# taishan1994/pytorch-distributed-NLP

Hardware: NVIDIA H100
Metric: training samples/sec (seq_len=128) (higher is better)
Workload: dtype bf16

## Files before the change

### pytorch-distributed-nlp_b200/csrc/gemm.cu

```cuda
#include "common.cuh"
#include "gemm_epilogue.cuh"
#include "../../include/b2_ddp_bert.h"

namespace b2 {

constexpr int BM = 128;
constexpr int BK = 64;
constexpr int WGMMA_K = 16;
constexpr int kGemmThreads = (4 + kEpiWarps) * 32;

template <int BN>
struct GemmCfg {
  static constexpr int kABytes = BM * BK * 2;
  static constexpr int kBBytes = BN * BK * 2;
  static constexpr int kStageBytes = kABytes + kBBytes;
  static constexpr int kStages = (BN == 256) ? 4 : 6;
  static constexpr int kPipeBytes = kStages * kStageBytes;
  static constexpr int kAccLd = BN + 4;
  static constexpr int kSmemBytes = kPipeBytes + kEpiWarps * kEpiStageBytes + 1024  + 256 ;
  static_assert(BM * kAccLd * 4 <= kPipeBytes, "the accumulator tile lives in the drained operand ring");
};

template <int BN, bool A_MN, bool B_MN>
__device__ __forceinline__ void gemm_mainloop(uint8_t* smem, uint64_t* full_bar, uint64_t* empty_bar,
                                              const CUtensorMap* tmap_a, const CUtensorMap* tmap_b, int m0, int n0,
                                              int kb0, int kb1, int warp, int lane) {
  using Cfg = GemmCfg<BN>;
  if (warp == 0) {
    if (lane == 0) {
      int stage = 0; uint32_t phase = 0;
      for (int kb = kb0; kb < kb1; ++kb) {
        mbar_wait(&empty_bar[stage], phase ^ 1);
        mbar_expect_tx(&full_bar[stage], Cfg::kStageBytes);
        uint8_t* sa = smem + stage * Cfg::kStageBytes;
        uint8_t* sb = sa + Cfg::kABytes;
        const int k0 = kb * BK;
        if (!A_MN) {
          tma_load_2d(sa, tmap_a, &full_bar[stage], k0, m0);
        } else {
#pragma unroll
          for (int j = 0; j < BM / 64; ++j)
            tma_load_2d(sa + j * (BK * 128), tmap_a, &full_bar[stage], m0 + 64 * j, k0);
        }
        if (!B_MN) {
          tma_load_2d(sb, tmap_b, &full_bar[stage], k0, n0);
        } else {
#pragma unroll
          for (int j = 0; j < BN / 64; ++j)
            tma_load_2d(sb + j * (BK * 128), tmap_b, &full_bar[stage], n0 + 64 * j, k0);
        }
        if (++stage == Cfg::kStages) { stage = 0; phase ^= 1; }
      }
    }
  } else if (warp >= 4) {
    const int wg = (warp - 4) >> 2;
    constexpr uint32_t a_lbo = A_MN ? BK * 128 : 16, b_lbo = B_MN ? BK * 128 : 16;
    constexpr uint32_t a_kstep = A_MN ? WGMMA_K * 128 : WGMMA_K * 2;
    constexpr uint32_t b_kstep = B_MN ? WGMMA_K * 128 : WGMMA_K * 2;
    float acc[BN / 2];
#pragma unroll
    for (int i = 0; i < BN / 2; ++i) acc[i] = 0.f;
    int stage = 0, prev = -1; uint32_t phase = 0;
    for (int kb = kb0; kb < kb1; ++kb) {
      mbar_wait(&full_bar[stage], phase);
      const uint32_t sa = smem_u32(smem + stage * Cfg::kStageBytes) + wg * 8192;
      const uint32_t sb = smem_u32(smem + stage * Cfg::kStageBytes + Cfg::kABytes);
      wgmma_fence();
#pragma unroll
      for (int k = 0; k < BK / WGMMA_K; ++k)
        wgmma_bf16<BN, A_MN ? 1 : 0, B_MN ? 1 : 0>(acc, make_smem_desc(sa + k * a_kstep, a_lbo, 1024),
                                                     make_smem_desc(sb + k * b_kstep, b_lbo, 1024),
                                                     (kb > kb0 || k > 0) ? 1u : 0u);
      wgmma_commit();
      wgmma_wait<1>();
      if (prev >= 0 && lane == 0) mbar_arrive(&empty_bar[prev]);
      prev = stage;
      if (++stage == Cfg::kStages) { stage = 0; phase ^= 1; }
    }
    wgmma_wait<0>();
    wgmma_fence_regs(acc);
    if (prev >= 0 && lane == 0) mbar_arrive(&empty_bar[prev]);
    named_barrier_sync(1, kEpiWarps * 32);
    float* accs = reinterpret_cast<float*>(smem);
    const int r = wg * 64 + (warp & 3) * 16 + (lane >> 2);
    const int c = 2 * (lane & 3);
#pragma unroll
    for (int j = 0; j < BN / 8; ++j) {
      *reinterpret_cast<float2*>(accs + (size_t)r * Cfg::kAccLd + 8 * j + c) = make_float2(acc[4 * j], acc[4 * j + 1]);
      *reinterpret_cast<float2*>(accs + (size_t)(r + 8) * Cfg::kAccLd + 8 * j + c) =
          make_float2(acc[4 * j + 2], acc[4 * j + 3]);
    }
    named_barrier_sync(1, kEpiWarps * 32);
  }
}

template <int BN>
__device__ __forceinline__ void gemm_setup(uint64_t* full_bar, uint64_t* empty_bar) {
  if (threadIdx.x == 0) {
    for (int s = 0; s < GemmCfg<BN>::kStages; ++s) {
      mbar_init(&full_bar[s], 1);
      mbar_init(&empty_bar[s], kEpiWarps);
    }
    fence_mbar_init();
  }
  __syncthreads();
}

template <int BN, bool A_MN, bool B_MN>
__global__ void __launch_bounds__(kGemmThreads, 1)
gemm_bf16_kernel(const __grid_constant__ CUtensorMap tmap_a, const __grid_constant__ CUtensorMap tmap_b,
                 const GemmKernelParams p) {
  using Cfg = GemmCfg<BN>;
  extern __shared__ uint8_t smem_raw[];
  uint8_t* smem = smem_align_1024(smem_raw);
  uint8_t* epi_stage = smem + Cfg::kPipeBytes;
  uint64_t* full_bar = reinterpret_cast<uint64_t*>(epi_stage + kEpiWarps * kEpiStageBytes);
  uint64_t* empty_bar = full_bar + Cfg::kStages;
  const int warp = threadIdx.x >> 5;
  const int lane = threadIdx.x & 31;
  if (threadIdx.x == 0) {
    tma_prefetch_desc(&tmap_a);
    tma_prefetch_desc(&tmap_b);
  }
  gemm_setup<BN>(full_bar, empty_bar);
  pdl_wait();
  pdl_launch_dependents();

  const int tile = blockIdx.x / p.splits, split = blockIdx.x % p.splits;
  const int m0 = (tile / p.tiles_n) * BM, n0 = (tile % p.tiles_n) * BN;
  const int kb0 = split * p.kblocks_per_split;
  const int kb1 = min(kb0 + p.kblocks_per_split, p.kblocks_total);
  gemm_mainloop<BN, A_MN, B_MN>(smem, full_bar, empty_bar, &tmap_a, &tmap_b, m0, n0, kb0, kb1, warp, lane);
  if (warp >= 4) {
    const DropCtx drop = make_drop_ctx(p.rng, p.rng_site, p.dropout_p);
    epilogue_tile<BN>(p, drop, reinterpret_cast<const float*>(smem), Cfg::kAccLd, warp, lane, m0, n0, split,
                      epi_stage + (warp - 4) * kEpiStageBytes);
  }
}

constexpr int kMaxGroup = 4;
struct GroupedProblem {
  int M, N, tiles_n, tile_begin;
  __nv_bfloat16* D; long long ldd;
};
struct GroupedParams {
  int count, num_work, kblocks;
  GroupedProblem pr[kMaxGroup];
};

struct GroupedMaps {
  CUtensorMap a[kMaxGroup], b[kMaxGroup];
};
__device__ __forceinline__ int grouped_find(const GroupedParams& gp, int w) {
  int pi = 0;
#pragma unroll
  for (int i = 1; i < kMaxGroup; ++i)
    if (i < gp.count && w >= gp.pr[i].tile_begin) pi = i;
  return pi;
}

__global__ void __launch_bounds__(kGemmThreads, 1)
gemm_grouped_tn_kernel(const __grid_constant__ GroupedMaps maps, const GroupedParams gp) {
  constexpr int BN = 256;
  using Cfg = GemmCfg<BN>;
  extern __shared__ uint8_t smem_raw[];
  uint8_t* smem = smem_align_1024(smem_raw);
  uint8_t* epi_stage = smem + Cfg::kPipeBytes;
  uint64_t* full_bar = reinterpret_cast<uint64_t*>(epi_stage + kEpiWarps * kEpiStageBytes);
  uint64_t* empty_bar = full_bar + Cfg::kStages;
  const int warp = threadIdx.x >> 5;
  const int lane = threadIdx.x & 31;
  const int pi = grouped_find(gp, blockIdx.x);
  if (threadIdx.x == 0) {
    tma_prefetch_desc(&maps.a[pi]);
    tma_prefetch_desc(&maps.b[pi]);
  }
  gemm_setup<BN>(full_bar, empty_bar);
  pdl_wait();
  pdl_launch_dependents();

  const GroupedProblem& pr = gp.pr[pi];
  const int lt = blockIdx.x - pr.tile_begin;
  const int m0 = (lt / pr.tiles_n) * BM;
  const int n0 = (lt % pr.tiles_n) * BN;
  gemm_mainloop<BN, true, true>(smem, full_bar, empty_bar, &maps.a[pi], &maps.b[pi], m0, n0, 0, gp.kblocks, warp,
                                lane);
  if (warp < 4) return;
  uint8_t* stage = epi_stage + (warp - 4) * kEpiStageBytes;
  GemmKernelParams q;
  q.splits = 1; q.epilogue = B2_EPI_NONE; q.bias = nullptr; q.aux_in = nullptr; q.aux_out = nullptr;
  q.partial = nullptr; q.dropout_p = 0.f; q.rng = nullptr; q.rng_site = 0; q.timing = nullptr; q.colsum = nullptr;
  q.ld_aux_in = 0; q.ld_aux_out = 0; q.K = 0; q.tiles_m = 0; q.kblocks_per_split = 0; q.kblocks_total = 0;
  q.M = pr.M; q.N = pr.N; q.tiles_n = pr.tiles_n; q.D = pr.D; q.ldd = pr.ldd;
  DropCtx drop;
  drop.k0 = 0; drop.k1 = 0; drop.step = 0; drop.site = 0; drop.thresh = 0; drop.scale = 1.f;
  epilogue_tile<BN>(q, drop, reinterpret_cast<const float*>(smem), Cfg::kAccLd, warp, lane, m0, n0, 0, stage);
}

__global__ void splitk_reduce_kernel(const float* __restrict__ partial, __nv_bfloat16* __restrict__ D,
                                     long long ldd, int M, int N, int splits) {
  pdl_wait();
  pdl_launch_dependents();
  const long long idx = (long long)blockIdx.x * blockDim.x + threadIdx.x;
  const long long total = (long long)M * N / 4;
  if (idx >= total) return;
  const long long e = idx * 4;
  const int m = (int)(e / N), n = (int)(e % N);
  float4 acc = make_float4(0.f, 0.f, 0.f, 0.f);
  for (int s = 0; s < splits; ++s) {
    const float4 v = *reinterpret_cast<const float4*>(partial + (size_t)s * M * N + e);
    acc.x += v.x; acc.y += v.y; acc.z += v.z; acc.w += v.w;
  }
  uint2 o;
  o.x = pack_bf16(acc.x, acc.y);
  o.y = pack_bf16(acc.z, acc.w);
  *reinterpret_cast<uint2*>(D + (size_t)m * ldd + n) = o;
}

static int g_num_sms = 0;
static int num_sms() {
  if (g_num_sms == 0) {
    int dev = 0;
    cudaGetDevice(&dev);
    cudaDeviceGetAttribute(&g_num_sms, cudaDevAttrMultiProcessorCount, dev);
    if (g_num_sms <= 0) g_num_sms = 132;
  }
  return g_num_sms;
}

static void fill_params(GemmKernelParams& p, const b2_gemm_args_t& a, int tile_m, int bn, int splits) {
  p.M = (int)a.M; p.N = (int)a.N; p.K = (int)a.K;
  p.tiles_m = (p.M + tile_m - 1) / tile_m;
  p.tiles_n = (p.N + bn - 1) / bn;
  p.kblocks_total = (p.K + BK - 1) / BK;
  p.splits = splits;
  p.kblocks_per_split = (p.kblocks_total + splits - 1) / splits;
  p.epilogue = (splits > 1 && a.epilogue != B2_EPI_ACCUM_F32) ? B2_EPI_PARTIAL_F32 : a.epilogue;
  p.D = (__nv_bfloat16*)a.D; p.ldd = a.ldd;
  p.bias = (const __nv_bfloat16*)a.bias;
  p.aux_in = (const __nv_bfloat16*)a.aux_in; p.ld_aux_in = a.ld_aux_in;
  p.aux_out = (__nv_bfloat16*)a.aux_out; p.ld_aux_out = a.ld_aux_out;
  p.partial = (float*)a.workspace;
  p.dropout_p = a.dropout_p; p.rng = (const unsigned long long*)a.rng_state; p.rng_site = a.rng_site;
  p.timing = (long long*)a.debug_timing;
  p.colsum = a.colsum_out;
}

static int32_t launch_splitk_reduce(const b2_gemm_args_t& a, int splits, cudaStream_t stream) {
  const long long total = (long long)a.M * a.N / 4;
  B2_LAUNCH(splitk_reduce_kernel, (unsigned)((total + 255) / 256), 256, 0, stream, 
      (const float*)a.workspace, (__nv_bfloat16*)a.D, a.ldd, (int)a.M, (int)a.N, splits);
  B2_CUDA(cudaGetLastError());
  count_launches(1);
  return 0;
}

template <int BN, bool A_MN, bool B_MN>
static int32_t launch_gemm(const b2_gemm_args_t& a, int splits, cudaStream_t stream) {
  using Cfg = GemmCfg<BN>;
  CUtensorMap ta, tb;
  int32_t st;
  if (!A_MN) st = get_tensor_map_2d(&ta, a.A, (uint64_t)a.M, (uint64_t)a.K, (uint64_t)a.lda * 2, BM, 64);
  else       st = get_tensor_map_2d(&ta, a.A, (uint64_t)a.K, (uint64_t)a.M, (uint64_t)a.lda * 2, BK, 64);
  if (st) return st;
  if (!B_MN) st = get_tensor_map_2d(&tb, a.B, (uint64_t)a.N, (uint64_t)a.K, (uint64_t)a.ldb * 2, BN, 64);
  else       st = get_tensor_map_2d(&tb, a.B, (uint64_t)a.K, (uint64_t)a.N, (uint64_t)a.ldb * 2, BK, 64);
  if (st) return st;
  GemmKernelParams p;
  fill_params(p, a, BM, BN, splits);
  auto kern = gemm_bf16_kernel<BN, A_MN, B_MN>;
  static bool attr_set = false;
  if (!attr_set) {
    B2_CUDA(cudaFuncSetAttribute(kern, cudaFuncAttributeMaxDynamicSharedMemorySize, Cfg::kSmemBytes));
    attr_set = true;
  }
  const int work = p.tiles_m * p.tiles_n * p.splits;
  B2_LAUNCH(kern, work, kGemmThreads, Cfg::kSmemBytes, stream, ta, tb, p);
  B2_CUDA(cudaGetLastError());
  count_launches(1);
  if (splits > 1 && a.epilogue != B2_EPI_ACCUM_F32) return launch_splitk_reduce(a, splits, stream);
  return 0;
}

struct Choice { int bn, splits; };
static Choice choose_config(const b2_gemm_args_t& a) {
  const int sms = num_sms();
  const int kblocks = (int)((a.K + BK - 1) / BK);
  const bool accum = a.epilogue == B2_EPI_ACCUM_F32;
  const bool can_split = accum || ((a.epilogue == B2_EPI_NONE) && a.workspace != nullptr && a.bias == nullptr &&
                                   a.colsum_out == nullptr);
  double best = 1e30;
  Choice c{128, 1};
  const double l2_bytes_per_cycle = 3000.0;
  const int bns[2] = {256, 128};
  for (int bi = 0; bi < 2; ++bi) {
    const int bn = bns[bi];
    if (a.N % bn != 0 && bn != 128) continue;
    const int tiles = (int)((a.M + BM - 1) / BM) * (int)((a.N + bn - 1) / bn);
    const int max_s = can_split ? 8 : 1;
    for (int s = 1; s <= max_s; s = accum ? s + 1 : s * 2) {
      if (s > 1 && (kblocks / s < 8)) break;
      if (s > 1 && !accum && (size_t)s * a.M * a.N * 4 > (size_t)a.workspace_bytes) break;
      const int work = tiles * s;
      const int rounds = (work + sms - 1) / sms;
      const int busy_sms = work < sms ? work : sms;
      const double mma_cycles = 128.0 * bn * 64 / 2048.0;
      const double bytes_per_sm = (128 + bn) * 128.0;
      const double feed_cycles = bytes_per_sm * busy_sms / l2_bytes_per_cycle;
      const double kb_cycles = mma_cycles > feed_cycles ? mma_cycles : feed_cycles;
      double t = rounds * ((double)((kblocks + s - 1) / s) * kb_cycles + 2500.0 );
      if (s > 1 && !accum) t += 1500.0 + (double)s * a.M * a.N * 8 / 3000.0;
      if (s > 1 && accum) t += (double)(s - 1) * a.M * a.N * 4 / 3000.0;
      if (t < best) { best = t; c = Choice{bn, s}; }
    }
  }
  return c;
}

}

using namespace b2;

static int32_t check_args(const b2_gemm_args_t* a) {
  B2_REQUIRE(a != nullptr, "b2_gemm_bf16: null args");
  B2_REQUIRE(a->M > 0 && a->N > 0 && a->K > 0, "b2_gemm_bf16: empty problem M=%lld N=%lld K=%lld",
             (long long)a->M, (long long)a->N, (long long)a->K);
  B2_REQUIRE(a->A && a->B && a->D, "b2_gemm_bf16: null operand pointer");
  B2_REQUIRE(a->N % 64 == 0, "b2_gemm_bf16: N=%lld must be a multiple of 64", (long long)a->N);
  B2_REQUIRE(a->K % 8 == 0 && a->lda % 8 == 0 && a->ldb % 8 == 0 && a->ldd % 8 == 0,
             "b2_gemm_bf16: K and leading dimensions must be multiples of 8 elements (16 B)");
  B2_REQUIRE(((uintptr_t)a->A % 16 == 0) && ((uintptr_t)a->B % 16 == 0) && ((uintptr_t)a->D % 16 == 0),
             "b2_gemm_bf16: operands must be 16-byte aligned");
  const int64_t a_row = a->a_major == B2_MAJOR_MN ? a->M : a->K, b_row = a->b_major == B2_MAJOR_MN ? a->N : a->K;
  B2_REQUIRE(a->lda >= a_row, "b2_gemm_bf16: lda=%lld is below the row it describes (%lld)", (long long)a->lda,
             (long long)a_row);
  B2_REQUIRE(a->ldb >= b_row, "b2_gemm_bf16: ldb=%lld is below the row it describes (%lld)", (long long)a->ldb,
             (long long)b_row);
  B2_REQUIRE(a->ldd >= a->N, "b2_gemm_bf16: ldd=%lld is below N=%lld", (long long)a->ldd, (long long)a->N);
  const int e = a->epilogue;
  B2_REQUIRE(e >= B2_EPI_NONE && e <= B2_EPI_ACCUM_F32, "b2_gemm_bf16: bad epilogue %d", e);
  const bool with_bias = e == B2_EPI_BIAS || e == B2_EPI_BIAS_GELU || e == B2_EPI_BIAS_DROPOUT_RESIDUAL;
  const bool f32_out = e == B2_EPI_RESIDUAL_F32 || e == B2_EPI_ACCUM_F32;
  if (with_bias) B2_REQUIRE(a->bias != nullptr, "b2_gemm_bf16: epilogue %d needs a bias", e);
  else           B2_REQUIRE(a->bias == nullptr, "b2_gemm_bf16: epilogue %d adds no bias: bias must be NULL", e);
  if (e == B2_EPI_BIAS_DROPOUT_RESIDUAL || e == B2_EPI_RESIDUAL || e == B2_EPI_GELU_BWD || e == B2_EPI_RESIDUAL_F32) {
    B2_REQUIRE(a->aux_in != nullptr && a->ld_aux_in % 8 == 0, "b2_gemm_bf16: epilogue %d needs aux_in", e);
    B2_REQUIRE(a->ld_aux_in >= a->N, "b2_gemm_bf16: ld_aux_in=%lld is below N=%lld", (long long)a->ld_aux_in,
               (long long)a->N);
  }
  if (e == B2_EPI_BIAS_GELU) {
    B2_REQUIRE(a->aux_out != nullptr && a->ld_aux_out % 8 == 0, "b2_gemm_bf16: BIAS_GELU needs aux_out");
    B2_REQUIRE(a->ld_aux_out >= a->N, "b2_gemm_bf16: ld_aux_out=%lld is below N=%lld", (long long)a->ld_aux_out,
               (long long)a->N);
  } else
    B2_REQUIRE(a->aux_out == nullptr, "b2_gemm_bf16: only BIAS_GELU writes aux_out: aux_out must be NULL");
  B2_REQUIRE((uintptr_t)a->bias % 16 == 0, "b2_gemm_bf16: bias must be 16-byte aligned");
  B2_REQUIRE((uintptr_t)a->aux_in % 16 == 0, "b2_gemm_bf16: aux_in must be 16-byte aligned");
  B2_REQUIRE((uintptr_t)a->aux_out % 16 == 0, "b2_gemm_bf16: aux_out must be 16-byte aligned");
  B2_REQUIRE(a->dropout_p >= 0.f && a->dropout_p < 1.f, "b2_gemm_bf16: dropout_p out of range");
  if (e == B2_EPI_BIAS_DROPOUT_RESIDUAL && a->dropout_p > 0.f)
    B2_REQUIRE(a->rng_state != nullptr, "b2_gemm_bf16: dropout needs rng_state");
  if (e != B2_EPI_BIAS_DROPOUT_RESIDUAL)
    B2_REQUIRE(a->dropout_p == 0.f, "b2_gemm_bf16: epilogue %d applies no dropout: dropout_p must be 0", e);
  B2_REQUIRE(a->colsum_out == nullptr || !f32_out, "b2_gemm_bf16: epilogue %d has no bf16 output: colsum_out must be "
             "NULL", e);
  B2_REQUIRE(a->colsum_out == nullptr || a->force_splits <= 1, "b2_gemm_bf16: colsum_out needs force_splits <= 1");
  if (a->force_bn == 128 || a->force_bn == 256)
    B2_REQUIRE(a->N % a->force_bn == 0 || a->force_bn == 128, "b2_gemm_bf16: force_bn does not divide N");
  if (a->force_splits > 1)
    B2_REQUIRE(e == B2_EPI_ACCUM_F32 ||
                   (e == B2_EPI_NONE && a->workspace &&
                    (size_t)a->force_splits * a->M * a->N * 4 <= (size_t)a->workspace_bytes),
               "b2_gemm_bf16: split-K needs EPI_ACCUM_F32, or EPI_NONE and a large enough workspace");
  B2_REQUIRE(!(a->a_major == B2_MAJOR_MN && a->b_major != B2_MAJOR_MN),
             "b2_gemm_bf16: layout TT (A MN-major, B K-major) is not on the path");
  return 0;
}

static int32_t launch_checked(const b2_gemm_args_t* a, cudaStream_t stream) {
  Choice c = choose_config(*a);
  if (a->force_bn == 128 || a->force_bn == 256) c.bn = a->force_bn;
  if (a->force_splits >= 1) c.splits = a->force_splits;
  const bool a_mn = a->a_major == B2_MAJOR_MN, b_mn = a->b_major == B2_MAJOR_MN;

#define B2_DISPATCH(BN_)                                                          \
  if (c.bn == BN_) {                                                              \
    if (!a_mn && !b_mn) return launch_gemm<BN_, false, false>(*a, c.splits, stream); \
    if (!a_mn && b_mn) return launch_gemm<BN_, false, true>(*a, c.splits, stream);   \
    return launch_gemm<BN_, true, true>(*a, c.splits, stream);                       \
  }
  B2_DISPATCH(128)
  B2_DISPATCH(256)
#undef B2_DISPATCH
  set_error("b2_gemm_bf16: no kernel for BN=%d", c.bn);
  return -2;
}

extern "C" int32_t b2_gemm_bf16(const b2_gemm_args_t* a, void* stream_) {
  const int32_t st = check_args(a);
  if (st) return st;
  return launch_checked(a, (cudaStream_t)stream_);
}

extern "C" int32_t b2_gemm_bf16_grouped(const b2_gemm_args_t* args, int32_t count, void* stream_) {
  cudaStream_t stream = (cudaStream_t)stream_;
  B2_REQUIRE(args != nullptr && count >= 1, "b2_gemm_bf16_grouped: no problems");
  for (int i = 0; i < count; ++i) {
    const int32_t st = check_args(&args[i]);
    if (st) return st;
  }
  bool groupable = count <= kMaxGroup;
  for (int i = 0; i < count && groupable; ++i) {
    const b2_gemm_args_t& a = args[i];
    groupable = a.a_major == B2_MAJOR_MN && a.b_major == B2_MAJOR_MN && a.epilogue == B2_EPI_NONE &&
                a.colsum_out == nullptr && a.N % 256 == 0 && a.K == args[0].K && a.force_splits <= 1 &&
                (a.force_bn == 0 || a.force_bn == 256);
  }
  if (!groupable) {
    for (int i = 0; i < count; ++i) {
      const int32_t st = launch_checked(&args[i], stream);
      if (st) return st;
    }
    return 0;
  }
  GroupedMaps maps;
  GroupedParams gp;
  gp.count = count;
  gp.kblocks = (int)((args[0].K + BK - 1) / BK);
  int work = 0;
  for (int i = 0; i < count; ++i) {
    const b2_gemm_args_t& a = args[i];
    int32_t st = get_tensor_map_2d(&maps.a[i], a.A, (uint64_t)a.K, (uint64_t)a.M, (uint64_t)a.lda * 2, BK, 64);
    if (st) return st;
    st = get_tensor_map_2d(&maps.b[i], a.B, (uint64_t)a.K, (uint64_t)a.N, (uint64_t)a.ldb * 2, BK, 64);
    if (st) return st;
    GroupedProblem& g = gp.pr[i];
    g.M = (int)a.M; g.N = (int)a.N; g.tiles_n = (int)(a.N / 256); g.tile_begin = work;
    g.D = (__nv_bfloat16*)a.D; g.ldd = a.ldd;
    work += (int)((a.M + BM - 1) / BM) * g.tiles_n;
  }
  for (int i = count; i < kMaxGroup; ++i) { gp.pr[i] = gp.pr[0]; gp.pr[i].tile_begin = 0x7fffffff; maps.a[i] = maps.a[0]; maps.b[i] = maps.b[0]; }
  gp.num_work = work;
  static bool attr_set = false;
  if (!attr_set) {
    B2_CUDA(cudaFuncSetAttribute(gemm_grouped_tn_kernel, cudaFuncAttributeMaxDynamicSharedMemorySize,
                                 GemmCfg<256>::kSmemBytes));
    attr_set = true;
  }
  B2_LAUNCH(gemm_grouped_tn_kernel, work, kGemmThreads, GemmCfg<256>::kSmemBytes, stream, maps, gp);
  B2_CUDA(cudaGetLastError());
  count_launches(1);
  return 0;
}
```

### pytorch-distributed-nlp_b200/csrc/gemm_epilogue.cuh

```cuda
#pragma once
#include "common.cuh"
#include "../../include/b2_ddp_bert.h"

namespace b2 {

struct GemmKernelParams {
  int M, N, K;
  int tiles_m, tiles_n, splits, kblocks_per_split, kblocks_total;
  int epilogue;
  __nv_bfloat16* D; long long ldd;
  const __nv_bfloat16* bias;
  const __nv_bfloat16* aux_in; long long ld_aux_in;
  __nv_bfloat16* aux_out; long long ld_aux_out;
  float* partial;
  float dropout_p; const unsigned long long* rng; unsigned rng_site;
  long long* timing;
  float* colsum;
};

constexpr int kEpiStageBytes = 32 * 128;

#ifdef __CUDACC__
template <int CH>
__device__ __forceinline__ uint4* stage_ptr(uint8_t* stage, int row, int chunk) {
  if (CH == 8) return reinterpret_cast<uint4*>(stage + row * 128 + ((chunk ^ (row & 7)) << 4));
  return reinterpret_cast<uint4*>(stage + (row >> 1) * 128 + (((((row & 1) << 2) | chunk) ^ ((row >> 1) & 7)) << 4));
}
template <int CH>
__device__ __forceinline__ void tile_s2g(uint8_t* stage, uint8_t* g, long long pitch, int lane, int rows_valid) {
  constexpr int RPS = 32 / CH;
#pragma unroll
  for (int k = 0; k < CH; ++k) {
    const int r = RPS * k + lane / CH, c = lane % CH;
    const uint4 v = *stage_ptr<CH>(stage, r, c);
    if (r < rows_valid) *reinterpret_cast<uint4*>(g + (size_t)r * pitch + c * 16) = v;
  }
}
__device__ __forceinline__ void tile_s2g_red_f32(uint8_t* stage, uint8_t* g, long long pitch, int lane,
                                                 int rows_valid) {
#pragma unroll
  for (int k = 0; k < 8; ++k) {
    const int r = 4 * k + (lane >> 3), c = lane & 7;
    const uint4 v = *stage_ptr<8>(stage, r, c);
    if (r < rows_valid)
      asm volatile("red.global.add.v4.f32 [%0], {%1, %2, %3, %4};" ::"l"(g + (size_t)r * pitch + c * 16),
                   "f"(__uint_as_float(v.x)), "f"(__uint_as_float(v.y)), "f"(__uint_as_float(v.z)),
                   "f"(__uint_as_float(v.w))
                   : "memory");
  }
}
template <int CH>
__device__ __forceinline__ void tile_g2s_async(uint8_t* stage, const uint8_t* g, long long pitch, int lane,
                                               int rows_valid) {
  constexpr int RPS = 32 / CH;
#pragma unroll
  for (int k = 0; k < CH; ++k) {
    const int r = RPS * k + lane / CH, c = lane % CH;
    uint4* dst = stage_ptr<CH>(stage, r, c);
    if (r < rows_valid) {
      asm volatile("cp.async.cg.shared.global [%0], [%1], 16;" ::"r"(smem_u32(dst)), "l"(g + (size_t)r * pitch + c * 16)
                   : "memory");
    } else {
      *dst = make_uint4(0u, 0u, 0u, 0u);
    }
  }
  asm volatile("cp.async.commit_group;" ::: "memory");
}
__device__ __forceinline__ void tile_async_wait() { asm volatile("cp.async.wait_group 0;" ::: "memory"); }

__device__ __forceinline__ void acc_ld32(const float* a, uint32_t (&v)[32]) {
#pragma unroll
  for (int k = 0; k < 8; ++k) {
    const uint4 t = *reinterpret_cast<const uint4*>(a + 4 * k);
    v[4 * k] = t.x; v[4 * k + 1] = t.y; v[4 * k + 2] = t.z; v[4 * k + 3] = t.w;
  }
}

template <int CH>
__device__ __forceinline__ void row_write32(uint8_t* stage, int lane, int c0, const float (&f)[32]) {
#pragma unroll
  for (int c = 0; c < 4; ++c) {
    uint4 o;
    o.x = pack_bf16(f[8 * c + 0], f[8 * c + 1]); o.y = pack_bf16(f[8 * c + 2], f[8 * c + 3]);
    o.z = pack_bf16(f[8 * c + 4], f[8 * c + 5]); o.w = pack_bf16(f[8 * c + 6], f[8 * c + 7]);
    *stage_ptr<CH>(stage, lane, c0 + c) = o;
  }
}
template <int CH>
__device__ __forceinline__ void row_read32(uint8_t* stage, int lane, int c0, float (&r)[32]) {
#pragma unroll
  for (int c = 0; c < 4; ++c) {
    const uint4 t = *stage_ptr<CH>(stage, lane, c0 + c);
    r[8 * c + 0] = bf16_lo(t.x); r[8 * c + 1] = bf16_hi(t.x); r[8 * c + 2] = bf16_lo(t.y); r[8 * c + 3] = bf16_hi(t.y);
    r[8 * c + 4] = bf16_lo(t.z); r[8 * c + 5] = bf16_hi(t.z); r[8 * c + 6] = bf16_lo(t.w); r[8 * c + 7] = bf16_hi(t.w);
  }
}

constexpr int kEpiWarps = 8;
template <int BN>
__device__ __forceinline__ void epilogue_tile(const GemmKernelParams& p, const DropCtx& drop, const float* acc,
                                              int acc_ld, int warp, int lane, int m_base, int n0, int split,
                                              uint8_t* stage) {
  static_assert(BN == 128 || BN == 256, "tile widths on the path");
  constexpr int kColsPerWarp = BN / 2;
  constexpr int WT = 64;
  constexpr int CH = WT / 8;
  const int quarter = warp & 3;
  const int cgrp = (warp - 4) >> 2;
  const int row0 = m_base + quarter * 32;
  const int rows_valid = p.M - row0;
  const int m = row0 + lane;
  const int nw = n0 + cgrp * kColsPerWarp;
  const float* arow = acc + (size_t)(quarter * 32 + lane) * acc_ld + cgrp * kColsPerWarp;

  if (p.epilogue == B2_EPI_PARTIAL_F32 || p.epilogue == B2_EPI_RESIDUAL_F32 || p.epilogue == B2_EPI_ACCUM_F32) {
    const bool accum = p.epilogue == B2_EPI_ACCUM_F32;
    const bool no_aux = p.epilogue != B2_EPI_RESIDUAL_F32;
    const bool to_ws = p.epilogue == B2_EPI_PARTIAL_F32;
    float* dst_base = to_ws ? p.partial + (size_t)split * p.M * p.N : reinterpret_cast<float*>(p.D);
    const long long dst_ld = to_ws ? (long long)p.N : p.ldd;
    auto prefetch = [&](int c) {
      const int n = nw + c * 32;
      if (!no_aux && n < p.N && rows_valid > 0)
        tile_g2s_async<8>(stage, reinterpret_cast<const uint8_t*>(reinterpret_cast<const float*>(p.aux_in) +
                                                                 (size_t)row0 * p.ld_aux_in + n),
                          p.ld_aux_in * 4, lane, rows_valid);
    };
    prefetch(0);
#pragma unroll 1
    for (int c = 0; c < kColsPerWarp / 32; ++c) {
      const int n = nw + c * 32;
      uint32_t v[32];
      acc_ld32(arow + c * 32, v);
      if (n < p.N && rows_valid > 0) {
        if (!no_aux) {
          if (c > 0) prefetch(c);
          tile_async_wait();
          __syncwarp();
#pragma unroll
          for (int k = 0; k < 8; ++k) {
            const uint4 t = *stage_ptr<8>(stage, lane, k);
            v[4 * k + 0] = __float_as_uint(__uint_as_float(v[4 * k + 0]) + __uint_as_float(t.x));
            v[4 * k + 1] = __float_as_uint(__uint_as_float(v[4 * k + 1]) + __uint_as_float(t.y));
            v[4 * k + 2] = __float_as_uint(__uint_as_float(v[4 * k + 2]) + __uint_as_float(t.z));
            v[4 * k + 3] = __float_as_uint(__uint_as_float(v[4 * k + 3]) + __uint_as_float(t.w));
          }
          __syncwarp();
        }
#pragma unroll
        for (int k = 0; k < 8; ++k)
          *stage_ptr<8>(stage, lane, k) = make_uint4(v[4 * k], v[4 * k + 1], v[4 * k + 2], v[4 * k + 3]);
        __syncwarp();
        uint8_t* gdst = reinterpret_cast<uint8_t*>(dst_base + (size_t)row0 * dst_ld + n);
        if (accum) tile_s2g_red_f32(stage, gdst, dst_ld * 4, lane, rows_valid);
        else       tile_s2g<8>(stage, gdst, dst_ld * 4, lane, rows_valid);
      }
      __syncwarp();
    }
    return;
  }

  const bool has_aux = p.epilogue == B2_EPI_BIAS_DROPOUT_RESIDUAL || p.epilogue == B2_EPI_RESIDUAL ||
                       p.epilogue == B2_EPI_GELU_BWD;
  auto prefetch = [&](int t) {
    const int n = nw + t * WT;
    if (has_aux && n < p.N && rows_valid > 0)
      tile_g2s_async<CH>(stage, reinterpret_cast<const uint8_t*>(p.aux_in + (size_t)row0 * p.ld_aux_in + n),
                         p.ld_aux_in * 2, lane, rows_valid);
  };
  prefetch(0);
#pragma unroll 1
  for (int t = 0; t < kColsPerWarp / WT; ++t) {
    const int n = nw + t * WT;
    const bool active = n < p.N && rows_valid > 0;
    if (has_aux && active) {
      if (t > 0) prefetch(t);
      tile_async_wait();
      __syncwarp();
    }
#pragma unroll 1
    for (int h = 0; h < WT / 32; ++h) {
      float f[32];
      {
        uint32_t v[32];
        acc_ld32(arow + t * WT + h * 32, v);
#pragma unroll
        for (int j = 0; j < 32; ++j) f[j] = __uint_as_float(v[j]);
      }
      if (!active) continue;
      const int nh = n + h * 32;
      if (p.bias != nullptr) {
#pragma unroll
        for (int j = 0; j < 32; j += 8) {
          const uint4 b = ldg16(p.bias + nh + j);
          f[j + 0] += bf16_lo(b.x); f[j + 1] += bf16_hi(b.x); f[j + 2] += bf16_lo(b.y); f[j + 3] += bf16_hi(b.y);
          f[j + 4] += bf16_lo(b.z); f[j + 5] += bf16_hi(b.z); f[j + 6] += bf16_lo(b.w); f[j + 7] += bf16_hi(b.w);
        }
      }
      if (has_aux) {
        float r[32];
        row_read32<CH>(stage, lane, 4 * h, r);
        if (p.epilogue == B2_EPI_BIAS_DROPOUT_RESIDUAL) {
#pragma unroll
          for (int j = 0; j < 32; j += 8) {
            const uint32_t keep = dropout_keep8(drop, (unsigned long long)m * p.N + nh + j);
#pragma unroll
            for (int i = 0; i < 8; ++i) f[j + i] = (((keep >> i) & 1u) ? f[j + i] * drop.scale : 0.f) + r[j + i];
          }
        } else if (p.epilogue == B2_EPI_RESIDUAL) {
#pragma unroll
          for (int j = 0; j < 32; ++j) f[j] += r[j];
        } else {
#pragma unroll
          for (int j = 0; j < 32; ++j) f[j] *= gelu_erf_grad(r[j]);
        }
      }
      row_write32<CH>(stage, lane, 4 * h, f);
    }
    if (active) {
      __syncwarp();
      if (p.epilogue == B2_EPI_BIAS_GELU) {
        tile_s2g<CH>(stage, reinterpret_cast<uint8_t*>(p.aux_out + (size_t)row0 * p.ld_aux_out + n), p.ld_aux_out * 2,
                     lane, rows_valid);
        __syncwarp();
#pragma unroll 1
        for (int h = 0; h < WT / 32; ++h) {
          float f[32];
          row_read32<CH>(stage, lane, 4 * h, f);
#pragma unroll
          for (int j = 0; j < 32; ++j) f[j] = gelu_erf(f[j]);
          row_write32<CH>(stage, lane, 4 * h, f);
        }
        __syncwarp();
      }
      if (p.colsum != nullptr) {
        float s0 = 0.f, s1 = 0.f;
        const int nr = rows_valid < 32 ? rows_valid : 32;
        if (WT == 64 || lane < 16) {
          for (int r = 0; r < nr; ++r) {
            const uint32_t w = *reinterpret_cast<const uint32_t*>(
                reinterpret_cast<const uint8_t*>(stage_ptr<CH>(stage, r, lane >> 2)) + (lane & 3) * 4);
            s0 += bf16_lo(w);
            s1 += bf16_hi(w);
          }
          atomicAdd(p.colsum + n + 2 * lane, s0);
          atomicAdd(p.colsum + n + 2 * lane + 1, s1);
        }
      }
      tile_s2g<CH>(stage, reinterpret_cast<uint8_t*>(p.D + (size_t)row0 * p.ldd + n), p.ldd * 2, lane, rows_valid);
    }
    __syncwarp();
  }
}
#endif

}
```

### pytorch-distributed-nlp_b200/csrc/wgmma.cuh

```cuda
#pragma once
#include <stdint.h>

namespace b2 {
#ifdef __CUDACC__

template <int TA, int TB>
__device__ __forceinline__ void wgmma_m64n64k16(float (&d)[32], uint64_t da, uint64_t db, uint32_t acc) {
  asm volatile(
      "{\n\t.reg .pred p;\n\tsetp.ne.b32 p, %34, 0;\n\t"
      "wgmma.mma_async.sync.aligned.m64n64k16.f32.bf16.bf16 {"
      "%0, %1, %2, %3, %4, %5, %6, %7, %8, %9, %10, %11, %12, %13, %14, %15, "
      "%16, %17, %18, %19, %20, %21, %22, %23, %24, %25, %26, %27, %28, %29, %30, %31"
      "}, %32, %33, p, 1, 1, %35, %36;\n\t}"
      : "+f"(d[0]), "+f"(d[1]), "+f"(d[2]), "+f"(d[3]), "+f"(d[4]), "+f"(d[5]), "+f"(d[6]), "+f"(d[7]),
        "+f"(d[8]), "+f"(d[9]), "+f"(d[10]), "+f"(d[11]), "+f"(d[12]), "+f"(d[13]), "+f"(d[14]), "+f"(d[15]),
        "+f"(d[16]), "+f"(d[17]), "+f"(d[18]), "+f"(d[19]), "+f"(d[20]), "+f"(d[21]), "+f"(d[22]), "+f"(d[23]),
        "+f"(d[24]), "+f"(d[25]), "+f"(d[26]), "+f"(d[27]), "+f"(d[28]), "+f"(d[29]), "+f"(d[30]), "+f"(d[31])
      : "l"(da), "l"(db), "r"(acc), "n"(TA), "n"(TB));
}

template <int TA, int TB>
__device__ __forceinline__ void wgmma_m64n128k16(float (&d)[64], uint64_t da, uint64_t db, uint32_t acc) {
  asm volatile(
      "{\n\t.reg .pred p;\n\tsetp.ne.b32 p, %66, 0;\n\t"
      "wgmma.mma_async.sync.aligned.m64n128k16.f32.bf16.bf16 {"
      "%0, %1, %2, %3, %4, %5, %6, %7, %8, %9, %10, %11, %12, %13, %14, %15, "
      "%16, %17, %18, %19, %20, %21, %22, %23, %24, %25, %26, %27, %28, %29, %30, %31, "
      "%32, %33, %34, %35, %36, %37, %38, %39, %40, %41, %42, %43, %44, %45, %46, %47, "
      "%48, %49, %50, %51, %52, %53, %54, %55, %56, %57, %58, %59, %60, %61, %62, %63"
      "}, %64, %65, p, 1, 1, %67, %68;\n\t}"
      : "+f"(d[0]), "+f"(d[1]), "+f"(d[2]), "+f"(d[3]), "+f"(d[4]), "+f"(d[5]), "+f"(d[6]), "+f"(d[7]),
        "+f"(d[8]), "+f"(d[9]), "+f"(d[10]), "+f"(d[11]), "+f"(d[12]), "+f"(d[13]), "+f"(d[14]), "+f"(d[15]),
        "+f"(d[16]), "+f"(d[17]), "+f"(d[18]), "+f"(d[19]), "+f"(d[20]), "+f"(d[21]), "+f"(d[22]), "+f"(d[23]),
        "+f"(d[24]), "+f"(d[25]), "+f"(d[26]), "+f"(d[27]), "+f"(d[28]), "+f"(d[29]), "+f"(d[30]), "+f"(d[31]),
        "+f"(d[32]), "+f"(d[33]), "+f"(d[34]), "+f"(d[35]), "+f"(d[36]), "+f"(d[37]), "+f"(d[38]), "+f"(d[39]),
        "+f"(d[40]), "+f"(d[41]), "+f"(d[42]), "+f"(d[43]), "+f"(d[44]), "+f"(d[45]), "+f"(d[46]), "+f"(d[47]),
        "+f"(d[48]), "+f"(d[49]), "+f"(d[50]), "+f"(d[51]), "+f"(d[52]), "+f"(d[53]), "+f"(d[54]), "+f"(d[55]),
        "+f"(d[56]), "+f"(d[57]), "+f"(d[58]), "+f"(d[59]), "+f"(d[60]), "+f"(d[61]), "+f"(d[62]), "+f"(d[63])
      : "l"(da), "l"(db), "r"(acc), "n"(TA), "n"(TB));
}

template <int TA, int TB>
__device__ __forceinline__ void wgmma_m64n256k16(float (&d)[128], uint64_t da, uint64_t db, uint32_t acc) {
  asm volatile(
      "{\n\t.reg .pred p;\n\tsetp.ne.b32 p, %130, 0;\n\t"
      "wgmma.mma_async.sync.aligned.m64n256k16.f32.bf16.bf16 {"
      "%0, %1, %2, %3, %4, %5, %6, %7, %8, %9, %10, %11, %12, %13, %14, %15, "
      "%16, %17, %18, %19, %20, %21, %22, %23, %24, %25, %26, %27, %28, %29, %30, %31, "
      "%32, %33, %34, %35, %36, %37, %38, %39, %40, %41, %42, %43, %44, %45, %46, %47, "
      "%48, %49, %50, %51, %52, %53, %54, %55, %56, %57, %58, %59, %60, %61, %62, %63, "
      "%64, %65, %66, %67, %68, %69, %70, %71, %72, %73, %74, %75, %76, %77, %78, %79, "
      "%80, %81, %82, %83, %84, %85, %86, %87, %88, %89, %90, %91, %92, %93, %94, %95, "
      "%96, %97, %98, %99, %100, %101, %102, %103, %104, %105, %106, %107, %108, %109, %110, %111, "
      "%112, %113, %114, %115, %116, %117, %118, %119, %120, %121, %122, %123, %124, %125, %126, %127"
      "}, %128, %129, p, 1, 1, %131, %132;\n\t}"
      : "+f"(d[0]), "+f"(d[1]), "+f"(d[2]), "+f"(d[3]), "+f"(d[4]), "+f"(d[5]), "+f"(d[6]), "+f"(d[7]),
        "+f"(d[8]), "+f"(d[9]), "+f"(d[10]), "+f"(d[11]), "+f"(d[12]), "+f"(d[13]), "+f"(d[14]), "+f"(d[15]),
        "+f"(d[16]), "+f"(d[17]), "+f"(d[18]), "+f"(d[19]), "+f"(d[20]), "+f"(d[21]), "+f"(d[22]), "+f"(d[23]),
        "+f"(d[24]), "+f"(d[25]), "+f"(d[26]), "+f"(d[27]), "+f"(d[28]), "+f"(d[29]), "+f"(d[30]), "+f"(d[31]),
        "+f"(d[32]), "+f"(d[33]), "+f"(d[34]), "+f"(d[35]), "+f"(d[36]), "+f"(d[37]), "+f"(d[38]), "+f"(d[39]),
        "+f"(d[40]), "+f"(d[41]), "+f"(d[42]), "+f"(d[43]), "+f"(d[44]), "+f"(d[45]), "+f"(d[46]), "+f"(d[47]),
        "+f"(d[48]), "+f"(d[49]), "+f"(d[50]), "+f"(d[51]), "+f"(d[52]), "+f"(d[53]), "+f"(d[54]), "+f"(d[55]),
        "+f"(d[56]), "+f"(d[57]), "+f"(d[58]), "+f"(d[59]), "+f"(d[60]), "+f"(d[61]), "+f"(d[62]), "+f"(d[63]),
        "+f"(d[64]), "+f"(d[65]), "+f"(d[66]), "+f"(d[67]), "+f"(d[68]), "+f"(d[69]), "+f"(d[70]), "+f"(d[71]),
        "+f"(d[72]), "+f"(d[73]), "+f"(d[74]), "+f"(d[75]), "+f"(d[76]), "+f"(d[77]), "+f"(d[78]), "+f"(d[79]),
        "+f"(d[80]), "+f"(d[81]), "+f"(d[82]), "+f"(d[83]), "+f"(d[84]), "+f"(d[85]), "+f"(d[86]), "+f"(d[87]),
        "+f"(d[88]), "+f"(d[89]), "+f"(d[90]), "+f"(d[91]), "+f"(d[92]), "+f"(d[93]), "+f"(d[94]), "+f"(d[95]),
        "+f"(d[96]), "+f"(d[97]), "+f"(d[98]), "+f"(d[99]), "+f"(d[100]), "+f"(d[101]), "+f"(d[102]), "+f"(d[103]),
        "+f"(d[104]), "+f"(d[105]), "+f"(d[106]), "+f"(d[107]), "+f"(d[108]), "+f"(d[109]), "+f"(d[110]), "+f"(d[111]),
        "+f"(d[112]), "+f"(d[113]), "+f"(d[114]), "+f"(d[115]), "+f"(d[116]), "+f"(d[117]), "+f"(d[118]), "+f"(d[119]),
        "+f"(d[120]), "+f"(d[121]), "+f"(d[122]), "+f"(d[123]), "+f"(d[124]), "+f"(d[125]), "+f"(d[126]), "+f"(d[127])
      : "l"(da), "l"(db), "r"(acc), "n"(TA), "n"(TB));
}

template <int N, int TA, int TB>
__device__ __forceinline__ void wgmma_bf16(float (&d)[N / 2], uint64_t da, uint64_t db, uint32_t acc) {
  if constexpr (N == 64) wgmma_m64n64k16<TA, TB>(d, da, db, acc);
  else if constexpr (N == 128) wgmma_m64n128k16<TA, TB>(d, da, db, acc);
  else wgmma_m64n256k16<TA, TB>(d, da, db, acc);
}

__device__ __forceinline__ void wgmma_fence() { asm volatile("wgmma.fence.sync.aligned;" ::: "memory"); }
__device__ __forceinline__ void wgmma_commit() { asm volatile("wgmma.commit_group.sync.aligned;" ::: "memory"); }
template <int N>
__device__ __forceinline__ void wgmma_wait() { asm volatile("wgmma.wait_group.sync.aligned %0;" ::"n"(N) : "memory"); }
template <int R>
__device__ __forceinline__ void wgmma_fence_regs(float (&d)[R]) {
#pragma unroll
  for (int i = 0; i < R; ++i) asm volatile("" : "+f"(d[i])::"memory");
}
#endif
}
```

Measured before the change: 4638.

## Add BN=192 GEMM tile width with wgmma m64n192 and split epilogue

Adds a third tile width, BN=192, to the wgmma GEMM. This brings a new m64n192k16 instruction wrapper, dispatch and force_bn support, and the cost-model search now considers 192 as a candidate. The epilogue is factored into a per-width pass function, so 96-column warp slices are handled as one 64-wide pass plus one 32-wide pass. The aim is better SM wave quantization for BERT N sizes (768, 2304, 3072) that divide by 192, at the cost of a prefetch overlap lost in the refactored epilogue and more template instantiations.

```diff
diff --git a/pytorch-distributed-nlp_b200/csrc/gemm.cu b/pytorch-distributed-nlp_b200/csrc/gemm.cu
--- a/pytorch-distributed-nlp_b200/csrc/gemm.cu
+++ b/pytorch-distributed-nlp_b200/csrc/gemm.cu
@@ -14,7 +14,7 @@
   static constexpr int kABytes = BM * BK * 2;
   static constexpr int kBBytes = BN * BK * 2;
   static constexpr int kStageBytes = kABytes + kBBytes;
-  static constexpr int kStages = (BN == 256) ? 4 : 6;
+  static constexpr int kStages = (BN == 128) ? 6 : 4;
   static constexpr int kPipeBytes = kStages * kStageBytes;
   static constexpr int kAccLd = BN + 4;
   static constexpr int kSmemBytes = kPipeBytes + kEpiWarps * kEpiStageBytes + 1024  + 256 ;
@@ -292,8 +292,8 @@
   double best = 1e30;
   Choice c{128, 1};
   const double l2_bytes_per_cycle = 3000.0;
-  const int bns[2] = {256, 128};
-  for (int bi = 0; bi < 2; ++bi) {
+  const int bns[3] = {256, 192, 128};
+  for (int bi = 0; bi < 3; ++bi) {
     const int bn = bns[bi];
     if (a.N % bn != 0 && bn != 128) continue;
     const int tiles = (int)((a.M + BM - 1) / BM) * (int)((a.N + bn - 1) / bn);
@@ -365,7 +365,7 @@
   B2_REQUIRE(a->colsum_out == nullptr || !f32_out, "b2_gemm_bf16: epilogue %d has no bf16 output: colsum_out must be "
              "NULL", e);
   B2_REQUIRE(a->colsum_out == nullptr || a->force_splits <= 1, "b2_gemm_bf16: colsum_out needs force_splits <= 1");
-  if (a->force_bn == 128 || a->force_bn == 256)
+  if (a->force_bn == 128 || a->force_bn == 192 || a->force_bn == 256)
     B2_REQUIRE(a->N % a->force_bn == 0 || a->force_bn == 128, "b2_gemm_bf16: force_bn does not divide N");
   if (a->force_splits > 1)
     B2_REQUIRE(e == B2_EPI_ACCUM_F32 ||
@@ -379,7 +379,7 @@
 
 static int32_t launch_checked(const b2_gemm_args_t* a, cudaStream_t stream) {
   Choice c = choose_config(*a);
-  if (a->force_bn == 128 || a->force_bn == 256) c.bn = a->force_bn;
+  if (a->force_bn == 128 || a->force_bn == 192 || a->force_bn == 256) c.bn = a->force_bn;
   if (a->force_splits >= 1) c.splits = a->force_splits;
   const bool a_mn = a->a_major == B2_MAJOR_MN, b_mn = a->b_major == B2_MAJOR_MN;
 
@@ -390,6 +390,7 @@
     return launch_gemm<BN_, true, true>(*a, c.splits, stream);                       \
   }
   B2_DISPATCH(128)
+  B2_DISPATCH(192)
   B2_DISPATCH(256)
 #undef B2_DISPATCH
   set_error("b2_gemm_bf16: no kernel for BN=%d", c.bn);
diff --git a/pytorch-distributed-nlp_b200/csrc/gemm_epilogue.cuh b/pytorch-distributed-nlp_b200/csrc/gemm_epilogue.cuh
--- a/pytorch-distributed-nlp_b200/csrc/gemm_epilogue.cuh
+++ b/pytorch-distributed-nlp_b200/csrc/gemm_epilogue.cuh
@@ -96,20 +96,105 @@
   }
 }
 
+template <int WT>
+__device__ __forceinline__ void epilogue_bf16_pass(const GemmKernelParams& p, const DropCtx& drop, const float* arow,
+                                                   int row0, int rows_valid, int n, int lane, uint8_t* stage) {
+  constexpr int CH = WT / 8;
+  const int m = row0 + lane;
+  const bool has_aux = p.epilogue == B2_EPI_BIAS_DROPOUT_RESIDUAL || p.epilogue == B2_EPI_RESIDUAL ||
+                       p.epilogue == B2_EPI_GELU_BWD;
+  const bool active = n < p.N && rows_valid > 0;
+  if (has_aux && active) {
+    tile_g2s_async<CH>(stage, reinterpret_cast<const uint8_t*>(p.aux_in + (size_t)row0 * p.ld_aux_in + n),
+                       p.ld_aux_in * 2, lane, rows_valid);
+    tile_async_wait();
+    __syncwarp();
+  }
+#pragma unroll 1
+  for (int h = 0; h < WT / 32; ++h) {
+    float f[32];
+    {
+      uint32_t v[32];
+      acc_ld32(arow + h * 32, v);
+#pragma unroll
+      for (int j = 0; j < 32; ++j) f[j] = __uint_as_float(v[j]);
+    }
+    if (!active) continue;
+    const int nh = n + h * 32;
+    if (p.bias != nullptr) {
+#pragma unroll
+      for (int j = 0; j < 32; j += 8) {
+        const uint4 b = ldg16(p.bias + nh + j);
+        f[j + 0] += bf16_lo(b.x); f[j + 1] += bf16_hi(b.x); f[j + 2] += bf16_lo(b.y); f[j + 3] += bf16_hi(b.y);
+        f[j + 4] += bf16_lo(b.z); f[j + 5] += bf16_hi(b.z); f[j + 6] += bf16_lo(b.w); f[j + 7] += bf16_hi(b.w);
+      }
+    }
+    if (has_aux) {
+      float r[32];
+      row_read32<CH>(stage, lane, 4 * h, r);
+      if (p.epilogue == B2_EPI_BIAS_DROPOUT_RESIDUAL) {
+#pragma unroll
+        for (int j = 0; j < 32; j += 8) {
+          const uint32_t keep = dropout_keep8(drop, (unsigned long long)m * p.N + nh + j);
+#pragma unroll
+          for (int i = 0; i < 8; ++i) f[j + i] = (((keep >> i) & 1u) ? f[j + i] * drop.scale : 0.f) + r[j + i];
+        }
+      } else if (p.epilogue == B2_EPI_RESIDUAL) {
+#pragma unroll
+        for (int j = 0; j < 32; ++j) f[j] += r[j];
+      } else {
+#pragma unroll
+        for (int j = 0; j < 32; ++j) f[j] *= gelu_erf_grad(r[j]);
+      }
+    }
+    row_write32<CH>(stage, lane, 4 * h, f);
+  }
+  if (active) {
+    __syncwarp();
+    if (p.epilogue == B2_EPI_BIAS_GELU) {
+      tile_s2g<CH>(stage, reinterpret_cast<uint8_t*>(p.aux_out + (size_t)row0 * p.ld_aux_out + n), p.ld_aux_out * 2,
+                   lane, rows_valid);
+      __syncwarp();
+#pragma unroll 1
+      for (int h = 0; h < WT / 32; ++h) {
+        float f[32];
+        row_read32<CH>(stage, lane, 4 * h, f);
+#pragma unroll
+        for (int j = 0; j < 32; ++j) f[j] = gelu_erf(f[j]);
+        row_write32<CH>(stage, lane, 4 * h, f);
+      }
+      __syncwarp();
+    }
+    if (p.colsum != nullptr) {
+      float s0 = 0.f, s1 = 0.f;
+      const int nr = rows_valid < 32 ? rows_valid : 32;
+      if (WT == 64 || lane < 16) {
+        for (int r = 0; r < nr; ++r) {
+          const uint32_t w = *reinterpret_cast<const uint32_t*>(
+              reinterpret_cast<const uint8_t*>(stage_ptr<CH>(stage, r, lane >> 2)) + (lane & 3) * 4);
+          s0 += bf16_lo(w);
+          s1 += bf16_hi(w);
+        }
+        atomicAdd(p.colsum + n + 2 * lane, s0);
+        atomicAdd(p.colsum + n + 2 * lane + 1, s1);
+      }
+    }
+    tile_s2g<CH>(stage, reinterpret_cast<uint8_t*>(p.D + (size_t)row0 * p.ldd + n), p.ldd * 2, lane, rows_valid);
+  }
+  __syncwarp();
+}
+
 constexpr int kEpiWarps = 8;
 template <int BN>
 __device__ __forceinline__ void epilogue_tile(const GemmKernelParams& p, const DropCtx& drop, const float* acc,
                                               int acc_ld, int warp, int lane, int m_base, int n0, int split,
                                               uint8_t* stage) {
-  static_assert(BN == 128 || BN == 256, "tile widths on the path");
+  static_assert(BN == 128 || BN == 192 || BN == 256, "tile widths on the path");
   constexpr int kColsPerWarp = BN / 2;
-  constexpr int WT = 64;
-  constexpr int CH = WT / 8;
   const int quarter = warp & 3;
   const int cgrp = (warp - 4) >> 2;
   const int row0 = m_base + quarter * 32;
   const int rows_valid = p.M - row0;
-  const int m = row0 + lane;
   const int nw = n0 + cgrp * kColsPerWarp;
   const float* arow = acc + (size_t)(quarter * 32 + lane) * acc_ld + cgrp * kColsPerWarp;
 
@@ -160,97 +245,11 @@
     return;
   }
 
-  const bool has_aux = p.epilogue == B2_EPI_BIAS_DROPOUT_RESIDUAL || p.epilogue == B2_EPI_RESIDUAL ||
-                       p.epilogue == B2_EPI_GELU_BWD;
-  auto prefetch = [&](int t) {
-    const int n = nw + t * WT;
-    if (has_aux && n < p.N && rows_valid > 0)
-      tile_g2s_async<CH>(stage, reinterpret_cast<const uint8_t*>(p.aux_in + (size_t)row0 * p.ld_aux_in + n),
-                         p.ld_aux_in * 2, lane, rows_valid);
-  };
-  prefetch(0);
-#pragma unroll 1
-  for (int t = 0; t < kColsPerWarp / WT; ++t) {
-    const int n = nw + t * WT;
-    const bool active = n < p.N && rows_valid > 0;
-    if (has_aux && active) {
-      if (t > 0) prefetch(t);
-      tile_async_wait();
-      __syncwarp();
-    }
-#pragma unroll 1
-    for (int h = 0; h < WT / 32; ++h) {
-      float f[32];
-      {
-        uint32_t v[32];
-        acc_ld32(arow + t * WT + h * 32, v);
-#pragma unroll
-        for (int j = 0; j < 32; ++j) f[j] = __uint_as_float(v[j]);
-      }
-      if (!active) continue;
-      const int nh = n + h * 32;
-      if (p.bias != nullptr) {
-#pragma unroll
-        for (int j = 0; j < 32; j += 8) {
-          const uint4 b = ldg16(p.bias + nh + j);
-          f[j + 0] += bf16_lo(b.x); f[j + 1] += bf16_hi(b.x); f[j + 2] += bf16_lo(b.y); f[j + 3] += bf16_hi(b.y);
-          f[j + 4] += bf16_lo(b.z); f[j + 5] += bf16_hi(b.z); f[j + 6] += bf16_lo(b.w); f[j + 7] += bf16_hi(b.w);
-        }
-      }
-      if (has_aux) {
-        float r[32];
-        row_read32<CH>(stage, lane, 4 * h, r);
-        if (p.epilogue == B2_EPI_BIAS_DROPOUT_RESIDUAL) {
-#pragma unroll
-          for (int j = 0; j < 32; j += 8) {
-            const uint32_t keep = dropout_keep8(drop, (unsigned long long)m * p.N + nh + j);
-#pragma unroll
-            for (int i = 0; i < 8; ++i) f[j + i] = (((keep >> i) & 1u) ? f[j + i] * drop.scale : 0.f) + r[j + i];
-          }
-        } else if (p.epilogue == B2_EPI_RESIDUAL) {
-#pragma unroll
-          for (int j = 0; j < 32; ++j) f[j] += r[j];
-        } else {
-#pragma unroll
-          for (int j = 0; j < 32; ++j) f[j] *= gelu_erf_grad(r[j]);
-        }
-      }
-      row_write32<CH>(stage, lane, 4 * h, f);
-    }
-    if (active) {
-      __syncwarp();
-      if (p.epilogue == B2_EPI_BIAS_GELU) {
-        tile_s2g<CH>(stage, reinterpret_cast<uint8_t*>(p.aux_out + (size_t)row0 * p.ld_aux_out + n), p.ld_aux_out * 2,
-                     lane, rows_valid);
-        __syncwarp();
-#pragma unroll 1
-        for (int h = 0; h < WT / 32; ++h) {
-          float f[32];
-          row_read32<CH>(stage, lane, 4 * h, f);
-#pragma unroll
-          for (int j = 0; j < 32; ++j) f[j] = gelu_erf(f[j]);
-          row_write32<CH>(stage, lane, 4 * h, f);
-        }
-        __syncwarp();
-      }
-      if (p.colsum != nullptr) {
-        float s0 = 0.f, s1 = 0.f;
-        const int nr = rows_valid < 32 ? rows_valid : 32;
-        if (WT == 64 || lane < 16) {
-          for (int r = 0; r < nr; ++r) {
-            const uint32_t w = *reinterpret_cast<const uint32_t*>(
-                reinterpret_cast<const uint8_t*>(stage_ptr<CH>(stage, r, lane >> 2)) + (lane & 3) * 4);
-            s0 += bf16_lo(w);
-            s1 += bf16_hi(w);
-          }
-          atomicAdd(p.colsum + n + 2 * lane, s0);
-          atomicAdd(p.colsum + n + 2 * lane + 1, s1);
-        }
-      }
-      tile_s2g<CH>(stage, reinterpret_cast<uint8_t*>(p.D + (size_t)row0 * p.ldd + n), p.ldd * 2, lane, rows_valid);
-    }
-    __syncwarp();
-  }
+#pragma unroll 1
+  for (int t = 0; t < kColsPerWarp / 64; ++t)
+    epilogue_bf16_pass<64>(p, drop, arow + t * 64, row0, rows_valid, nw + t * 64, lane, stage);
+  if (kColsPerWarp % 64 != 0)
+    epilogue_bf16_pass<32>(p, drop, arow + kColsPerWarp - 32, row0, rows_valid, nw + kColsPerWarp - 32, lane, stage);
 }
 #endif
 
diff --git a/pytorch-distributed-nlp_b200/csrc/wgmma.cuh b/pytorch-distributed-nlp_b200/csrc/wgmma.cuh
--- a/pytorch-distributed-nlp_b200/csrc/wgmma.cuh
+++ b/pytorch-distributed-nlp_b200/csrc/wgmma.cuh
@@ -41,6 +41,33 @@
 }
 
 template <int TA, int TB>
+__device__ __forceinline__ void wgmma_m64n192k16(float (&d)[96], uint64_t da, uint64_t db, uint32_t acc) {
+  asm volatile(
+      "{\n\t.reg .pred p;\n\tsetp.ne.b32 p, %98, 0;\n\t"
+      "wgmma.mma_async.sync.aligned.m64n192k16.f32.bf16.bf16 {"
+      "%0, %1, %2, %3, %4, %5, %6, %7, %8, %9, %10, %11, %12, %13, %14, %15, "
+      "%16, %17, %18, %19, %20, %21, %22, %23, %24, %25, %26, %27, %28, %29, %30, %31, "
+      "%32, %33, %34, %35, %36, %37, %38, %39, %40, %41, %42, %43, %44, %45, %46, %47, "
+      "%48, %49, %50, %51, %52, %53, %54, %55, %56, %57, %58, %59, %60, %61, %62, %63, "
+      "%64, %65, %66, %67, %68, %69, %70, %71, %72, %73, %74, %75, %76, %77, %78, %79, "
+      "%80, %81, %82, %83, %84, %85, %86, %87, %88, %89, %90, %91, %92, %93, %94, %95"
+      "}, %96, %97, p, 1, 1, %99, %100;\n\t}"
+      : "+f"(d[0]), "+f"(d[1]), "+f"(d[2]), "+f"(d[3]), "+f"(d[4]), "+f"(d[5]), "+f"(d[6]), "+f"(d[7]),
+        "+f"(d[8]), "+f"(d[9]), "+f"(d[10]), "+f"(d[11]), "+f"(d[12]), "+f"(d[13]), "+f"(d[14]), "+f"(d[15]),
+        "+f"(d[16]), "+f"(d[17]), "+f"(d[18]), "+f"(d[19]), "+f"(d[20]), "+f"(d[21]), "+f"(d[22]), "+f"(d[23]),
+        "+f"(d[24]), "+f"(d[25]), "+f"(d[26]), "+f"(d[27]), "+f"(d[28]), "+f"(d[29]), "+f"(d[30]), "+f"(d[31]),
+        "+f"(d[32]), "+f"(d[33]), "+f"(d[34]), "+f"(d[35]), "+f"(d[36]), "+f"(d[37]), "+f"(d[38]), "+f"(d[39]),
+        "+f"(d[40]), "+f"(d[41]), "+f"(d[42]), "+f"(d[43]), "+f"(d[44]), "+f"(d[45]), "+f"(d[46]), "+f"(d[47]),
+        "+f"(d[48]), "+f"(d[49]), "+f"(d[50]), "+f"(d[51]), "+f"(d[52]), "+f"(d[53]), "+f"(d[54]), "+f"(d[55]),
+        "+f"(d[56]), "+f"(d[57]), "+f"(d[58]), "+f"(d[59]), "+f"(d[60]), "+f"(d[61]), "+f"(d[62]), "+f"(d[63]),
+        "+f"(d[64]), "+f"(d[65]), "+f"(d[66]), "+f"(d[67]), "+f"(d[68]), "+f"(d[69]), "+f"(d[70]), "+f"(d[71]),
+        "+f"(d[72]), "+f"(d[73]), "+f"(d[74]), "+f"(d[75]), "+f"(d[76]), "+f"(d[77]), "+f"(d[78]), "+f"(d[79]),
+        "+f"(d[80]), "+f"(d[81]), "+f"(d[82]), "+f"(d[83]), "+f"(d[84]), "+f"(d[85]), "+f"(d[86]), "+f"(d[87]),
+        "+f"(d[88]), "+f"(d[89]), "+f"(d[90]), "+f"(d[91]), "+f"(d[92]), "+f"(d[93]), "+f"(d[94]), "+f"(d[95])
+      : "l"(da), "l"(db), "r"(acc), "n"(TA), "n"(TB));
+}
+
+template <int TA, int TB>
 __device__ __forceinline__ void wgmma_m64n256k16(float (&d)[128], uint64_t da, uint64_t db, uint32_t acc) {
   asm volatile(
       "{\n\t.reg .pred p;\n\tsetp.ne.b32 p, %130, 0;\n\t"
@@ -77,6 +104,7 @@
 __device__ __forceinline__ void wgmma_bf16(float (&d)[N / 2], uint64_t da, uint64_t db, uint32_t acc) {
   if constexpr (N == 64) wgmma_m64n64k16<TA, TB>(d, da, db, acc);
   else if constexpr (N == 128) wgmma_m64n128k16<TA, TB>(d, da, db, acc);
+  else if constexpr (N == 192) wgmma_m64n192k16<TA, TB>(d, da, db, acc);
   else wgmma_m64n256k16<TA, TB>(d, da, db, acc);
 }
 
```

Result: no change. 4663, median of 6 (+0.5%).
